# churchill-lab/alntools

Hardware: AMD Instinct MI355X
Metric: alignments/sec BAM->EC (100M PE reads, 8-hap) at 1/2/4/8 MI355X (higher is better)
Workload: dtype u32

## Files before the change

alntools_amd/csrc/ecb.hip:

```cpp
#include <hip/hip_runtime.h>

#include <algorithm>
#include <climits>
#include <cstddef>
#include <cstdarg>
#include <cstdio>
#include <cstring>
#include <cstdlib>
#include <memory>
#include <mutex>
#include <string>
#include <vector>

#include "../../include/ecb.h"

namespace {

typedef unsigned long long u64;
typedef unsigned int u32;
typedef unsigned short u16;

constexpr int TPB = 256;
constexpr u32 MAX_PROBE = 256;
constexpr u32 PENDING = 0xFFFFFFFFu;
// ... 8 lines not shown

constexpr u32 ERR_CONTRACT = 1u;
constexpr u32 ERR_RANGE = 2u;
constexpr u32 ERR_ARENA = 4u;
constexpr u32 ERR_QUEUE = 8u;
constexpr u32 ERR_INTERNAL = 16u;
constexpr u32 ERR_COUNT = 32u;

struct alignas(64) Slot {
    u64 lo;
    u32 n1;
    u32 off;
    u32 count;
    u32 first_inv;
    uint2 pair[INL];
};
static_assert(sizeof(Slot) == 64, "one EC per 64-byte line");
static_assert(offsetof(Slot, n1) == 8 && offsetof(Slot, off) == 12 && offsetof(Slot, count) == 16 && offsetof(Slot, first_inv) == 20,
              "k_count_bins reads {n1, off} and {count, first_inv} as 8-byte words");
struct Entry {
    u64 lo, reserved;
    u32 count, first_inv;
    u32 off, n;
};
static_assert(sizeof(Entry) == 32, "exchange format");

struct Counters {
    u64 all, valid;
    u64 arena_top;
    u64 n_queue;
    u64 n_queue_s[QSTRIPES];
    u64 n_ecs;
    u32 err;
    u32 full;
    u64 arena_reg[ARENA_REGIONS];
    u64 next_slice;
    u64 n_mismatch;
    u32 last_rid, pad_;
    u64 n_probe_tiles;
};

__host__ __device__ __forceinline__ u32 arena_regions(u64 arena_cap) { return (u32)(arena_cap >> 16 >= ARENA_REGIONS ? ARENA_REGIONS : (arena_cap >> 16 ? arena_cap >> 16 : 1)); }
__device__ __forceinline__ u64 arena_alloc(Counters* ctr, u64 arena_cap, u32 n, u32 hint) {
    const u32 R = arena_regions(arena_cap);
    const u64 per = arena_cap / R;
    for (u32 t = 0; t < R; ++t) {
        const u32 r = (hint + t) % R;
        const u64 at = atomicAdd(&ctr->arena_reg[r], (u64)n);
        if (at + n <= (u64)(r + 1) * per) return at;
    }
    return ~0ull;
}

__device__ __forceinline__ u32 fmix32(u32 h) {
    h ^= h >> 16; h *= 0x85EBCA6Bu;
    h ^= h >> 13; h *= 0xC2B2AE35u;
    h ^= h >> 16;
    return h;
}
__device__ __forceinline__ u64 pair_hash64(u32 locus, u32 mask) {
    const u32 h0 = fmix32(locus * 0x9E3779B1u + mask * 0x85EBCA77u + 0x7F4A7C15u);
    const u32 h1 = fmix32((h0 ^ locus) * 0xC2B2AE3Du + mask);
    return ((u64)h1 << 32) | h0;
}
__device__ __forceinline__ u64 finish_hash(u64 s0, u32 n) { return (s0 + ((u64)n << 32) + n) | 1ull; }

__device__ __forceinline__ bool rec_valid(u32 hf) {
    if (hf & 0x4u) return false;
    if (hf & 0x1u) {
        if ((hf & 0x80u) || !(hf & 0x2u) || (hf & (ECB_FLAG_MATE_OTHER_REF | ECB_FLAG_NEXT_POS_NEG))) return false;
    }
    return true;
}

enum { ST_NONE = 0, ST_LOOK, ST_HIT, ST_CREATED, ST_PENDING, ST_FULL, ST_OTHER, ST_STUCK };
enum { CMP_EQUAL = 0, CMP_DIFFERENT, CMP_INCOMPLETE, CMP_UNSURE };
struct SlotView { u32 n, off; uint2 p[INL]; };

__device__ __forceinline__ u64 fresh64(u64* p) { return atomicOr(p, 0ull); }
__device__ __forceinline__ void store_wt64(u64* p, u64 v) { __hip_atomic_store(p, v, __ATOMIC_RELAXED, __HIP_MEMORY_SCOPE_AGENT); }
__device__ __forceinline__ u64 pack2(uint2 v) { return ((u64)v.y << 32) | v.x; }
__device__ __forceinline__ uint2 unpack2(u64 v) { return make_uint2((u32)v, (u32)(v >> 32)); }
__device__ __forceinline__ void publish_key(Slot* s, u32 n1, u32 off) { store_wt64(reinterpret_cast<u64*>(&s->n1), ((u64)off << 32) | n1); }
__device__ __forceinline__ uint2 key_pair(const Slot& s, const uint2* arena, u32 i) { return i < INL ? s.pair[i] : arena[(u64)s.off + (i - INL)]; }
__device__ __forceinline__ uint2 key_pair_fresh(Slot* s, uint2* arena, u32 off, u32 i) {
    return unpack2(fresh64(reinterpret_cast<u64*>(i < INL ? &s->pair[i] : arena + ((u64)off + (i - INL)))));
}

__device__ __forceinline__ SlotView make_view(uint4 a, uint4 b, uint4 c, uint4 d) {
    SlotView v;
    v.n = a.z - 1u; v.off = a.w;
    v.p[0] = make_uint2(b.z, b.w); v.p[1] = make_uint2(c.x, c.y); v.p[2] = make_uint2(c.z, c.w);
    v.p[3] = make_uint2(d.x, d.y); v.p[4] = make_uint2(d.z, d.w);
    return v;
}
constexpr u32 RANKED_MAX = 16;
template <class F>
__device__ __forceinline__ void ranked_pairs(const SlotView& v, const uint2* arena, F&& emit) {
    const u32 sn = v.n;
    u32 X[RANKED_MAX], Y[RANKED_MAX];
#pragma unroll
    for (u32 i = 0; i < INL; ++i) { X[i] = i < sn ? v.p[i].x : 0xFFFFFFFFu; Y[i] = v.p[i].y; }
    if (sn <= INL) {
#pragma unroll
        for (u32 i = 0; i < INL; ++i) {
            u32 r = 0;
#pragma unroll
            for (u32 j = 0; j < INL; ++j) r += X[j] < X[i] ? 1u : 0u;
            if (i < sn) emit(r, X[i], Y[i]);
        }
    } else {
#pragma unroll
        for (u32 k = 0; k < RANKED_MAX - INL; ++k) {
            const uint2 t = INL + k < sn ? arena[(u64)v.off + k] : make_uint2(0xFFFFFFFFu, 0u);
            X[INL + k] = t.x; Y[INL + k] = t.y;
        }
#pragma unroll
        for (u32 i = 0; i < RANKED_MAX; ++i) {
            u32 r = 0;
#pragma unroll
            for (u32 j = 0; j < RANKED_MAX; ++j) r += X[j] < X[i] ? 1u : 0u;
            if (i < sn) emit(r, X[i], Y[i]);
        }
    }
}
constexpr u32 BIG_LDS = 2048;
template <class F>
__device__ __forceinline__ void ranked_pairs_wave(const Slot& s, const uint2* arena, u32 sn, u32* sx, u32 lane, F&& emit) {
    const bool in_lds = sn <= BIG_LDS;
    if (in_lds) {
        for (u32 i = lane; i < sn; i += 64) sx[i] = key_pair(s, arena, i).x;
        __builtin_amdgcn_fence(__ATOMIC_ACQ_REL, "wavefront");
        __builtin_amdgcn_wave_barrier();
    }
    for (u32 i = lane; i < sn; i += 64) {
        const uint2 pi = key_pair(s, arena, i);
        u32 r = 0;
        if (in_lds) {
            u32 j = 0;
            for (; j + 4u <= sn; j += 4u) {
                const uint4 v = *reinterpret_cast<const uint4*>(&sx[j]);
                r += (v.x < pi.x ? 1u : 0u) + (v.y < pi.x ? 1u : 0u) + (v.z < pi.x ? 1u : 0u) + (v.w < pi.x ? 1u : 0u);
            }
            for (; j < sn; ++j) r += sx[j] < pi.x ? 1u : 0u;
        } else {
            for (u32 j = 0; j < sn; ++j) r += key_pair(s, arena, j).x < pi.x;
        }
        emit(r, pi.x, pi.y);
    }
    if (in_lds) {
        __builtin_amdgcn_fence(__ATOMIC_ACQ_REL, "wavefront");
        __builtin_amdgcn_wave_barrier();
    }
}
template <class Cmp>
__device__ __forceinline__ int table_lookup(Slot* table, u64 cap_mask, u64 lo, u64& j, u32& probes, const Cmp& cmp, u32 abl = 0u, u32* first_inv_seen = nullptr) {
    for (; probes < MAX_PROBE; ++probes, j = (j + 1) & cap_mask) {
        Slot* s = table + j;
        const uint4* q = reinterpret_cast<const uint4*>(s);
        if (first_inv_seen) *first_inv_seen = 0u;
        uint4 a = q[0], b = a, c = a, d = a;
        if (!(abl & 16u)) { b = q[1]; c = q[2]; d = q[3]; }
        u64 clo = ((u64)a.y << 32) | a.x;
        if (clo == 0ull) {
            clo = atomicCAS(&s->lo, 0ull, lo);
            if (clo == 0ull) return ST_CREATED;
// ... 2283 lines not shown
int verify_pass(ecb_handle* h, const StreamPlan& P, const u32* d_rid, const u32* d_loc, const u32* d_hf, u64 n, u32 prev_rid, u64* n_long, u32 tw) {
    RCCHK(launch_stream(h, SV_VERIFY, P, d_rid, d_loc, d_hf, nullptr, n, prev_rid, nullptr, 0, 0));
    RCCHK(sync_counters(h));
    return run_deferred(h, d_rid, d_loc, d_hf, n, true, tw, n_long);
}
int verify_batch(ecb_handle* h, const u32* d_rid, const u32* d_loc, const u32* d_hf, u64 n, u32 prev_rid, u64* n_mismatch, u64* n_long, u32 tw = 512u) {
    StreamPlan P;
    RCCHK(plan_stream(h, n, &P, SV_VERIFY));
    u64 nq = 0;
    if (const int rc = verify_pass(h, P, d_rid, d_loc, d_hf, n, prev_rid, &nq, tw); rc != ECB_OK) {
        if (h->hctr.err) {
            const std::string refusal = h->err;
            HIPCHK(h, hipMemsetAsync(&h->ctr->err, 0, sizeof(u32), h->stream));
            HIPCHK(h, hipMemsetAsync(&h->ctr->n_queue, 0, (1 + QSTRIPES) * sizeof(u64), h->stream));
            h->hctr.err = 0; h->hctr.n_queue = 0;
            h->err = refusal;
        }
        return rc;
    }
    *n_mismatch = h->hctr.n_mismatch;
    *n_long = nq;
    HIPCHK(h, hipMemsetAsync(&h->ctr->n_queue, 0, (1 + QSTRIPES) * sizeof(u64), h->stream));
    h->hctr.n_queue = 0;
    return ECB_OK;
}

int build_batch(ecb_handle* h, const u32* d_rid, const u32* d_loc, const u32* d_hf, const int* d_pos, u64 n, u32 tw, bool* launched) {
    if (n == 0) return ECB_OK;
    const bool hinted = h->reads_hint != 0;
    u32 last_rid = 0;
    u64 reads_after = std::max<u64>(h->reads_hint, h->run.n_reads);
    if (!hinted) {
        HIPCHK(h, hipMemcpyAsync(&last_rid, d_rid + rec_at(n - 1, tw), sizeof(u32), hipMemcpyDeviceToHost, h->stream));
        HIPCHK(h, hipStreamSynchronize(h->stream));
        reads_after = (u64)(u32)(last_rid + 1u);
        if (reads_after < h->run.n_reads) return fail(h, ECB_ERR_CONTRACT, "read_id went backwards across pushes");
    }
    RCCHK(ensure_read_slot(h, reads_after));
    h->run.reads_hi = reads_after;
    while (h->n_ecs() * 2 > h->cap) { RCCHK(grow_table(h, h->cap * 4)); }
    const StreamVariant v = pick_variant(h, n);
    StreamPlan P;
    RCCHK(plan_stream(h, n, &P, v));
    u64* timing = nullptr;
#ifdef ECB_TIMING
    HIPCHK(h, hipMalloc(&timing, 8 * sizeof(u64)));
    HIPCHK(h, hipMemset(timing, 0, 8 * sizeof(u64)));
#endif
    h->ctr_synced = false;
    *launched = true;
    const u64 probe_before = h->hctr.n_probe_tiles;
    int rc = ECB_OK;
    for (u32 launch = 0;; ++launch) {
        rc = launch_stream(h, v, P, d_rid, d_loc, d_hf, d_pos, n, h->run.prev_rid, d_rid + rec_at(n - 1, tw), launch, launch ? 0 : n, timing);
        if (rc != ECB_OK) break;
        rc = sync_counters(h);
        if (h->prof) {
            float ms = 0; hipEventElapsedTime(&ms, h->ev0, h->ev1);
            h->prof_ms += ms; h->prof_launches += 1;
        }
        if (rc != ECB_OK) break;
        const bool parked = h->hctr.full != 0;
        rc = run_deferred(h, d_rid, d_loc, d_hf, n, false, tw);
        if (rc != ECB_OK) break;
        if (!parked) break;
        rc = grow_table(h, h->cap * 4);
        if (rc != ECB_OK) break;
    }
#ifdef ECB_TIMING
    {
        u64 t[8];
        hipMemcpy(t, timing, sizeof(t), hipMemcpyDeviceToHost); hipFree(timing);
        static const char* nm[8] = {"(a) filter+heads", "tile decisions", "prefetch issue+clear+geometry", "(b) LDS tables", "hash entries", "(c) lookup", "publish/settle/slot stores", "-"};
        u64 tot = 0; for (int i = 0; i < 7; ++i) tot += t[i];
        fprintf(stderr, "[ecb timing] %llu waves, clocks per wave:", (unsigned long long)P.slices);
        for (int i = 0; i < 7; ++i) fprintf(stderr, "  %s %.0f (%.1f%%)", nm[i], (double)t[i] / P.slices, 100.0 * t[i] / std::max<u64>(tot, 1));
        fprintf(stderr, "  tile visits on the probe-on path %llu of %llu tiles", (unsigned long long)t[7], (unsigned long long)((n + WT - 1) / WT));
        fprintf(stderr, "\n");
    }
#endif
    RCCHK(rc);
    {
        const u64 tiles = (n + WT - 1) / WT, on_path = h->hctr.n_probe_tiles - probe_before;
        if (on_path * 4 > tiles) h->par_stream = true; else if (on_path * 16 < tiles) h->par_stream = false;
    }
    if (h->prof) h->prof_records += n;
    if (h->cfg.flags & ECB_F_VERIFY) {
        u64 bad = 0, nl = 0;
        RCCHK(verify_batch(h, d_rid, d_loc, d_hf, n, h->run.prev_rid, &bad, &nl, tw));
        h->run.n_mismatch += bad;
        if (bad) return fail(h, ECB_ERR_VERIFY, "exactness pass: %llu read(s) of this batch sit in an EC whose key is not their target set", (unsigned long long)bad);
    }
    if (hinted) {
        last_rid = h->hctr.last_rid;
        reads_after = (u64)(u32)(last_rid + 1u);
        if (reads_after < h->run.n_reads) return fail(h, ECB_ERR_CONTRACT, "read_id went backwards across pushes");
    }
    h->run.prev_rid = last_rid;
    h->run.n_reads = reads_after;
    h->run.records_pushed += n;
    return ECB_OK;
}
int process_batch(ecb_handle* h, const u32* d_rid, const u32* d_loc, const u32* d_hf, const int* d_pos, u64 n, u32 tw = 512u) {
    bool launched = false;
    const int rc = build_batch(h, d_rid, d_loc, d_hf, d_pos, n, tw, &launched);
    return launched ? run_refused(h, rc) : rc;
}

int ensure_staging(ecb_handle* h, u64 need) {
    if (need <= h->st_cap) return ECB_OK;
    h->st_loc = h->st_hf = nullptr; h->st_pos = nullptr; h->st_cap = 0;
    const u64 cap = std::max<u64>(need, h->cfg.max_batch_records);
    const u64 stride = (cap * sizeof(u32) + (2ull << 20) - 1) / (2ull << 20) * (2ull << 20) / sizeof(u32);
    const bool rg = (h->cfg.flags & ECB_F_RANGES) != 0;
    HIPCHK(h, h->st_rid.alloc((rg ? 4 : 3) * stride * sizeof(u32)));
    h->st_cap = cap;
    h->st_loc = h->st_rid + stride; h->st_hf = h->st_rid + 2 * stride;
    if (rg) h->st_pos = reinterpret_cast<int*>(h->st_rid + 3 * stride);
    return ECB_OK;
}

int stage_and_process(ecb_handle* h, const u32* rid, const u32* loc, const u32* hf, const int* pos, u64 m) {
    const u64 nc = h->run.c_rid.size();
    const u64 n = nc + m;
    if (!n) return ECB_OK;
    RCCHK(ensure_staging(h, n));
    const bool rg = (h->cfg.flags & ECB_F_RANGES) != 0;
    const struct { void* st; const void *carry, *window; } streams[4] = {
        {h->st_rid, h->run.c_rid.data(), rid}, {h->st_loc, h->run.c_loc.data(), loc}, {h->st_hf, h->run.c_hf.data(), hf}, {h->st_pos, h->run.c_pos.data(), pos}};
    for (int w = 0; w < 2; ++w)
        for (int i = 0; i < (rg ? 4 : 3) && (w ? m : nc); ++i)
            HIPCHK(h, hipMemcpyAsync((u32*)streams[i].st + (w ? nc : 0), w ? streams[i].window : streams[i].carry, (w ? m : nc) * 4, hipMemcpyHostToDevice, h->stream));
    HIPCHK(h, hipStreamSynchronize(h->stream));
    h->run.c_rid.clear(); h->run.c_loc.clear(); h->run.c_hf.clear(); h->run.c_pos.clear();
    return process_batch(h, h->st_rid, h->st_loc, h->st_hf, rg ? h->st_pos : nullptr, n);
}

int excl_scan_dev(ecb_handle* h, const u32* in, u64 n, u32* out, u64* d_total, u32 stride = 1, u32* last32 = nullptr) {
    u32* sums = nullptr;
    POOL(h, P_SUMS, sums, scan_words(n));
    HIPCHK(h, scan_launch(h->stream, in, n, out, sums, d_total, stride, last32));
    return ECB_OK;
}
int excl_scan(ecb_handle* h, const u32* in, u64 n, u32* out, u64* total) {
    u64* d_tot = nullptr;
    POOL(h, P_TOTALS, d_tot, 8);
    RCCHK(excl_scan_dev(h, in, n, out, d_tot + 7));
    HIPCHK(h, hipMemcpyAsync(total, d_tot + 7, sizeof(u64), hipMemcpyDeviceToHost, h->stream));
    HIPCHK(h, hipStreamSynchronize(h->stream));
    return ECB_OK;
}

struct SortBufs {
    u64* k[2];
    u32* v[2];
    int at = 0;
    u64* keys() const { return k[at]; }
    u32* vals() const { return v[at]; }
    u64* spare_keys() const { return k[at ^ 1]; }
    u32* spare_vals() const { return v[at ^ 1]; }
};
struct SortScratch { u32 *hist, *offs; u64* d_word; };
inline u64 rs_tiles(u64 n) { return std::max<u64>(1, (n + RS_TILE - 1) / RS_TILE); }
constexpr u64 RS_AUX_WORDS = 2 * RS_MAX_PASSES * 256 + 64;
inline u64 rs_words(u64 n) { return std::max<u64>(256 * rs_tiles(n), RS_AUX_WORDS); }
hipError_t radix_sort_pairs64(hipStream_t st, SortBufs& b, u64 n, const SortScratch& sc, u64 bit_mask = ~0ull) {
    b.at = 0;
// ... 3120 lines not shown
```

alntools_amd/csrc/k_stream.inc:

```
constexpr bool KS_SHORT = ECB_KS_SHORT != 0;
#ifndef ECB_KS_PAR
#define ECB_KS_PAR 0
#endif
constexpr bool KS_PAR = ECB_KS_PAR != 0;
static_assert(!(KS_PAR && KS_SHORT), "one or the other");
constexpr u32 KBITS = KS_SHORT ? 25 : 26;
constexpr u32 KMASK = (1u << KBITS) - 1u;
constexpr int WMAXR = KS_SHORT ? 128 : 64;
#ifndef ECB_WAVES_PER_SIMD
#define ECB_WAVES_PER_SIMD 5
#endif
#ifndef ECB_LGMAX
#define ECB_LGMAX 6
#endif
#ifndef ECB_EST_MUL
#define ECB_EST_MUL 4
#endif
constexpr int WAVES_PER_SIMD = KS_SHORT ? 4 : ECB_WAVES_PER_SIMD;
constexpr int LGMAX = KS_SHORT ? 7 : ECB_LGMAX;
static_assert(LGMAX >= 0 && (1 << LGMAX) <= WMAXR && KBITS + LGMAX <= 32, "a read's index within the pass: the bits of an LDS key above KBITS");
constexpr int CMAX = KS_SHORT ? 64 : 80;
#ifndef ECB_TSLOTS
#define ECB_TSLOTS (ECB_WAVES_PER_SIMD > 4 ? 640 : 896)
#endif
constexpr int TSLOTS = KS_SHORT ? 1280 : ECB_TSLOTS;
constexpr int TBASE = KS_SHORT ? 1024 : 512;
constexpr int TAB_BYTES = KS_SHORT ? TSLOTS * 4 + 2048 : TSLOTS * 8;
static_assert((TSLOTS == 896 || TSLOTS == 640 || TSLOTS == 1280) && WT + CMAX < TSLOTS && TAB_BYTES % (16 * 64) == 0 && (!KS_SHORT || TSLOTS <= 2048), "home regions / a free slot / clear loop");
constexpr u32 SBITS = KS_SHORT ? 11 : 10;
constexpr u32 SMASK = (1u << SBITS) - 1u;
static_assert(TSLOTS <= (1 << SBITS) && (KS_SHORT || SBITS + LGMAX <= 16), "ent[] packs slot | read << SBITS into 16 bits (128 reads: the slot alone, the read is in the table's key)");
struct alignas(16) WaveLds {
#ifdef ECB_TAB_INTERLEAVED
    uint2 tab[TSLOTS];
#else
    u32 tkey[TSLOTS];
    u32 tmask[KS_SHORT ? 512 : TSLOTS];
#endif
    u64 acc[WMAXR];
    uint2 carry[CMAX];
    unsigned short ent[WT + CMAX];
    unsigned short npair[WMAXR];
    u32 ws[8];
};
static_assert(sizeof(WaveLds) * NWAVE * WAVES_PER_SIMD <= 160 * 1024, "WAVES_PER_SIMD workgroups per CU");
__device__ __forceinline__ u64 ws_get64(const WaveLds& L, int i) {
    const u32 lo = (u32)__builtin_amdgcn_readfirstlane((int)L.ws[i]), hi = (u32)__builtin_amdgcn_readfirstlane((int)L.ws[i + 1]);
    return ((u64)hi << 32) | lo;
}
__device__ __forceinline__ void ws_put64(WaveLds& L, int i, u64 v, u32 lane) { if (lane == 0) { L.ws[i] = (u32)v; L.ws[i + 1] = (u32)(v >> 32); } }
#ifdef ECB_TAB_INTERLEAVED
__device__ __forceinline__ u32* tab_key(WaveLds& L, u32 q) { return &L.tab[q].x; }
__device__ __forceinline__ void tab_or(WaveLds& L, u32 q, u32 bits) { static_assert(!KS_SHORT, "byte masks: split arrays only"); atomicOr(&L.tab[q].y, bits); }
__device__ __forceinline__ uint2 tab_get(const WaveLds& L, u32 q) { return L.tab[q]; }
__device__ __forceinline__ uint4* tab_base(WaveLds& L) { return reinterpret_cast<uint4*>(L.tab); }
#else
__device__ __forceinline__ u32* tab_key(WaveLds& L, u32 q) { return &L.tkey[q]; }
__device__ __forceinline__ void tab_or(WaveLds& L, u32 q, u32 bits) {
    if constexpr (KS_SHORT) atomicOr(&L.tmask[q >> 2], bits << ((q & 3u) * 8u)); else atomicOr(&L.tmask[q], bits);
}
__device__ __forceinline__ uint2 tab_get(const WaveLds& L, u32 q) {
    if constexpr (KS_SHORT) return make_uint2(L.tkey[q], (L.tmask[q >> 2] >> ((q & 3u) * 8u)) & 0xFFu);
    else return make_uint2(L.tkey[q], L.tmask[q]);
}
__device__ __forceinline__ uint4* tab_base(WaveLds& L) { return reinterpret_cast<uint4*>(L.tkey); }
#endif
struct HomeGeo { u32 fmul, g; };
__device__ __forceinline__ u32 pack_lgf(u32 lg) {
    const u32 g = (u32)(KS_SHORT ? 10 : 9) - lg;
    u32 x = 1u << 16, f = 0;
#pragma unroll
    for (int i = 0; i < 6; ++i) { f += x; x >>= g; }
    return f | (lg << 24);
}
__device__ __forceinline__ HomeGeo home_geo(u32 lgf) {
    HomeGeo H;
    H.fmul = lgf;
    H.g = (u32)(KS_SHORT ? 10 : 9) - (lgf >> 24);
    return H;
}
__device__ __forceinline__ u32 home_off(u32 key, const HomeGeo& H) { return __builtin_amdgcn_ubfe(__umul24(key, H.fmul), 16u, H.g); }
__device__ __forceinline__ u32 next_slot(u32 key, u32 q, u32 it) {
    if (it == 0u) return __umulhi(key * 0x9E3779B1u, (u32)TSLOTS);
    constexpr u32 ODD_FACTOR = TSLOTS == 896 ? 7u : 5u;
    u32 s = 1u + 2u * ((key >> 5) & 31u);
    if (s % ODD_FACTOR == 0u) s += 2u;
    q += s;
    return q >= (u32)TSLOTS ? q - (u32)TSLOTS : q;
}
__device__ __forceinline__ u32 probe_slot(u32 key, u32 it) {
    u32 q = __umulhi(key * 0x9E3779B1u, (u32)TSLOTS);
    if (it != 0u) {
        constexpr u32 ODD_FACTOR = TSLOTS == 896 ? 7u : 5u;
        u32 s = 1u + 2u * ((key >> 5) & 31u);
        if (s % ODD_FACTOR == 0u) s += 2u;
        q = (q + it * s) % (u32)TSLOTS;
    }
    return q;
}

struct LdsSetCmp {
    const WaveLds* L;
    u32 home, tag, np;
// ... 106 lines not shown
            const u32 key = tag | (pr.x + 1u);
            u32 q = home + home_off(pr.x + 1u, H);
            bool found = false;
            for (u32 it = 0; it < (u32)TSLOTS; ++it) {
                const uint2 t = tab_get(*L, q);
                if (t.x == key) { found = t.y == pr.y; break; }
                if (t.x == 0u) break;
                q = next_slot(key, q, it);
            }
            if (!found) return CMP_DIFFERENT;
        }
        return CMP_EQUAL;
    }
};

template <bool VERIFY, bool RANGES = false>
__global__ __launch_bounds__(TPB, RANGES ? (WAVES_PER_SIMD < 4 ? WAVES_PER_SIMD : 4) : WAVES_PER_SIMD) void k_stream(StreamArgs A) {
    __shared__ WaveLds wl[NWAVE];
    const u32 lane = threadIdx.x & 63u, w = threadIdx.x >> 6;
    WaveLds& L = wl[w];
    const u64 pw = (u64)blockIdx.x * NWAVE + w;
    const StreamCold* const C = A.cold;
    static_assert(WT == 512, "tile index = record index >> 9");
    u32 my_valid = 0, my_new = 0;
    u32 bad = 0;
    if (lane == 0) L.ws[7] = 0u;
    if (!VERIFY && lane == 0) { const u64* wa = C->wave_arena; const u64 ca = wa[2 * pw]; L.ws[2] = (u32)ca; L.ws[3] = (u32)(ca >> 32); L.ws[4] = (u32)wa[2 * pw + 1]; }
#ifdef ECB_TIMING
    u64 tacc[8] = {0, 0, 0, 0, 0, 0, 0, 0}, tlast = __builtin_readcyclecounter();
#endif
    auto clear_pass = [&](u32 ln) {
        uint4* z = tab_base(L);
        u32 zz;
        asm volatile("v_mov_b32 %0, 0" : "=v"(zz));
        const uint4 zv = make_uint4(zz, zz, zz, zz);
#pragma unroll
        for (int t = 0; t < TAB_BYTES / (16 * 64); ++t) z[t * 64 + ln] = zv;
        if constexpr (KS_SHORT) { reinterpret_cast<uint4*>(L.acc)[ln] = zv; reinterpret_cast<u32*>(L.npair)[ln] = zz; }
        else { *reinterpret_cast<uint2*>(&L.acc[ln]) = make_uint2(zz, zz); L.npair[ln] = (unsigned short)zz; }
    };
    clear_pass(lane);
    wave_sync();
  for (;;) {
    u32 wid = 0;
    if (lane == 0) wid = (u32)atomicAdd(&A.ctr->next_slice, 1ull);
    wid = (u32)__builtin_amdgcn_readfirstlane((int)wid);
    const u64 chunk = C->chunk;
    const u64 c0 = (u64)wid * chunk;
    if (c0 >= A.n) break;
    const u64 c1 = min(c0 + chunk, A.n);
    const u64 p = C->resume[2 * (u64)wid], counted0 = C->resume[2 * (u64)wid + 1];
    if (p >= A.n || p == ~0ull) continue;
    u32 tix = (u32)(p >> 9);
    const u32 c1t = (u32)((c1 + (u64)(WT - 1)) >> 9);
    const u32 last_t = (u32)((A.n - 1) >> 9);
    const u32 last_rel = (u32)(A.n - ((u64)last_t << 9));
    const u32 counted_t = (u32)((counted0 + (u64)(WT - 1)) >> 9);
    int p_rel = (int)(p - ((u64)tix << 9));
    u32 prev = p == 0 ? C->prev_rid : A.rid[rec_at(p - 1, A_TW(A))];
    u32 pb = prev + 1u, npend = 0, n_ent = 0;
    ws_put64(L, 5, p, lane);
    bool open = false;
    u32 carry_n = 0;
    u32 lgf = pack_lgf(LGMAX);
    bool revisit = false;
    TileRegs R;
    load_tile(A, (u64)tix << 9, min(((u64)tix << 9) + (u64)WT, A.n), lane, R);
    int r_pos[RANGES ? RPL : 1];
    if constexpr (RANGES) load_pos(A.pos, (u64)tix << 9, min(((u64)tix << 9) + (u64)WT, A.n), lane, r_pos);
    u32 parked = __hip_atomic_load(&A.ctr->full, __ATOMIC_RELAXED, __HIP_MEMORY_SCOPE_AGENT);
    asm volatile("" : "+v"(parked));
    bool slice_done = false;

    while (!slice_done) {
        if (__builtin_amdgcn_readfirstlane((int)parked)) break;
        u32 ln = lane;
        asm volatile("" : "+v"(ln));
        tix = (u32)__builtin_amdgcn_readfirstlane((int)tix);
        prev = (u32)__builtin_amdgcn_readfirstlane((int)prev);
        pb = (u32)__builtin_amdgcn_readfirstlane((int)pb);
        npend = (u32)__builtin_amdgcn_readfirstlane((int)npend);
        n_ent = (u32)__builtin_amdgcn_readfirstlane((int)n_ent);
        lgf = (u32)__builtin_amdgcn_readfirstlane((int)lgf);
        const u32 lg = lgf >> 24;
        const u32 gp = ((u32)TBASE >> lg) + (TSLOTS == 896 ? (256u >> lg) : 0u) + ((u32)(TBASE / 4) >> lg);
        const HomeGeo HG = home_geo(lgf);
        bool do_flush = false, again = false, more = false;
        bool preflush = false;
        bool taken = false;
        u32 parked_next = parked;
        u32 last_pos = 0xFFFFFFFFu;
        u32 last_rid = prev;
        u32 est = 64;
        const bool ends = tix == last_t;
        const bool own = tix < c1t;
        const int te_rel = ends ? (int)last_rel : WT;
        const bool count_tile = own && tix >= counted_t && !revisit;
        const bool plain = p_rel == 0 && te_rel == WT;
        u32 r_key[RPL], r_bit[RPL];
        u32 m_act = 0, m_head = 0;
        const u32 lim = own ? (1u << lg) : (open ? npend + 1u : 0u);
        const u32 rid_first = (u32)__builtin_amdgcn_readfirstlane((int)R.rr[0]), rid_last = (u32)__builtin_amdgcn_readlane((int)R.rr[RPL - 1], 63);
        const bool all_mine = rid_first - pb < lim && rid_last - pb < lim && rid_last >= rid_first;
        {
#pragma unroll
            for (int g = 0; g < NG; ++g) {
                const int i0 = g * 256 + 4 * (int)ln;
                const u32 up = lane_above(R.rr[4 * g + 3]);
                const u32 wrap = g == 0 ? prev : (u32)__builtin_amdgcn_readlane((int)R.rr[4 * (g > 0 ? g - 1 : 0) + 3], 63);
                u32 in4 = 0xFu, te4 = 0xFu;
                if (!plain) {
                    te4 = (1u << clamp04(te_rel - i0, 0, 4)) - 1u;
                    in4 = te4 & ~((1u << clamp04(p_rel - i0, 0, 4)) - 1u);
                }
                const u32 prev0 = ln == 0 ? wrap : up;
                u32 ok4 = 0, head4 = 0, hap_or = 0, mine4 = 0;
#pragma unroll
                for (int j = 3; j >= 0; --j) {
                    const u32 f = R.hh[4 * g + j];
                    const u32 pair_ok = ((f & 0x3082u) ^ 0x2u) - 1u;
                    const u32 ok31 = ~(f << 29) & (~(f << 31) | pair_ok);
                    ok4 = __builtin_amdgcn_alignbit(ok4, ok31, 31);
                }
#pragma unroll
                for (int par = 0; par < 2; ++par) {
                    if (__ballot((ok4 & (par ? 0xAu : 0x5u)) != 0u) != 0ull) {
#pragma unroll
                        for (int j = par; j < 4; j += 2) {
                            const int k = 4 * g + j;
                            const u32 f = R.hh[k];
                            const u32 step = R.rr[k] - (j == 0 ? prev0 : R.rr[k > 0 ? k - 1 : 0]);
                            const u32 relx = R.rr[k] - pb;
                            const u32 t = R.ll[k] + 1u;
                            r_key[k] = t | (relx << KBITS);
                            r_bit[k] = 1u << ((f >> ECB_HAP_SHIFT) & 31u);
                            hap_or |= ((t & ~KMASK) | f) & (u32)((int)(ok4 << (31 - j)) >> 31);
                            head4 |= (step & 1u) << j;
                            if (!all_mine) mine4 |= (relx < lim ? 1u : 0u) << j;
                        }
                        if constexpr (RANGES) {
                            if (!revisit) {
                                const u32 nl = C->n_loci, nh = C->n_haps;
                                int2* const rng = A.rng;
                                u32 sl[2]; int2 cur[2]; bool go[2];
#pragma unroll
                                for (int j = par; j < 4; j += 2) {
                                    const int k = 4 * g + j;
                                    const u32 lc = R.ll[k], hap = (R.hh[k] >> ECB_HAP_SHIFT) & 0xFFu;
                                    go[j >> 1] = ((ok4 >> j) & 1u) && lc < nl && hap < nh;
                                    sl[j >> 1] = lc * nh + hap;
                                    cur[j >> 1] = make_int2(0, 0);
                                    if (go[j >> 1]) cur[j >> 1] = rng[sl[j >> 1]];
                                }
#pragma unroll
                                for (int j = par; j < 4; j += 2) {
                                    const int ps = r_pos[RANGES ? 4 * g + j : 0];
                                    if (go[j >> 1] && ps < cur[j >> 1].x) atomicMin(&rng[sl[j >> 1]].x, ps);
                                    if (go[j >> 1] && ps > cur[j >> 1].y) atomicMax(&rng[sl[j >> 1]].y, ps);
                                }
                            }
                        }
                    } else {
#pragma unroll
                        for (int j = par; j < 4; j += 2) {
                            asm volatile("" : "=v"(r_key[4 * g + j])); asm volatile("" : "=v"(r_bit[4 * g + j]));
                        }
                    }
                }
                const u32 big = (u32)(R.rr[4 * g + 3] - prev0 != (u32)__popc(head4));
                if (count_tile) my_valid += __popc(ok4 & te4);
                ok4 &= in4; head4 &= in4;
                bad |= ((p_rel == 0 ? big : 0u) | (head4 & ~ok4)) ? ERR_CONTRACT : 0u;
                bad |= (hap_or >> (ECB_HAP_SHIFT + (KS_SHORT ? 3 : 5))) ? ERR_RANGE : 0u;
                m_act |= (all_mine ? ok4 : (ok4 & mine4)) << (4 * g); m_head |= head4 << (4 * g);
            }
        }
        TICK(0);
        if (__ballot(bad != 0u)) break;
        const u32 cnts = wave_sum((u32)__popc(m_head) | ((u32)__popc(m_act) << 16));
        const u32 nheads = cnts & 0xFFFFu, n_mine = cnts >> 16;
        last_rid = (u32)__builtin_amdgcn_readlane((int)R.rr[RPL - 1], 63);
        const u32 o1 = open ? 1u : 0u;
        const u32 n_new = own ? (prev + 1u + nheads) - (pb + npend + o1) : 0u;
        const u32 n_in = o1 + n_new;
        est = n_in;
        if (n_ent + carry_n + n_mine > (u32)(WT + CMAX)) { preflush = true; do_flush = true; }
        else {
        if (own) {
            if (npend + n_in > (1u << lg)) { again = true; npend = 1u << lg; open = false; }
            else if (n_in) { npend += ends ? n_in : n_in - 1u; open = !ends; }
        } else if (open && (nheads || ends)) { npend += 1u; open = false; }
        more = !ends && (tix + 1u < c1t || open);
        TICK(1);
        if (more || again) {
            u32 lp = ln;
#pragma unroll
            for (int k = 0; k < RPL; ++k) asm volatile("" : "+v"(lp) : "v"(r_key[k]), "v"(r_bit[k]));
            asm volatile("" : "+v"(lp) : "v"(m_act), "v"(m_head), "v"(bad), "v"(my_valid));
            const u64 nt = (u64)(again ? tix : tix + 1u) << 9;
            load_tile(A, nt, min(nt + (u64)WT, A.n), lp, R);
            if constexpr (RANGES) load_pos(A.pos, nt, min(nt + (u64)WT, A.n), lp, r_pos);
            parked_next = __hip_atomic_load(&A.ctr->full, __ATOMIC_RELAXED, __HIP_MEMORY_SCOPE_AGENT);
        }
        if (!again) {
            const u64 h1 = __ballot((m_head >> 4) != 0u), h0 = __ballot((m_head & 15u) != 0u);
            if (h1 | h0) {
                const u32 l = 63u - (u32)__builtin_clzll(h1 ? h1 : h0);
                const u32 bits = (u32)__builtin_amdgcn_readlane((int)m_head, (int)l);
                const u32 k = 31u - (u32)__builtin_clz(h1 ? bits & 0xF0u : bits & 0xFu);
                last_pos = (k & 3u) + (k >> 2) * 256u + 4u * l;
            }
            if (open && last_pos != 0xFFFFFFFFu) ws_put64(L, 0, ((u64)tix << 9) + last_pos, ln);
        }

        TICK(2);
        if (!ABL(A, 1u)) {
            const bool cin = carry_n != 0u;
            u32 q[RPL + 1], old[RPL + 1], act = m_act;
            u32 cb = 0;
            u32 c_key = 0, c_bit = 0;
            if (cin && ln < carry_n) { const uint2 cv = L.carry[ln]; c_key = cv.x; c_bit = cv.y; act |= 1u << RPL; }
#pragma unroll
            for (int h = 0; h < 2; ++h) {
                const u32 hmask = h ? 0x0AAu : 0x155u;
                if (__ballot((act & hmask) != 0u) == 0ull) continue;
#pragma unroll
                for (int k = h; k <= RPL; k += 2) {
                    const u32 key = k < RPL ? r_key[k < RPL ? k : 0] : c_key;
                    q[k] = (act >> k & 1u) ? (key >> KBITS) * gp + home_off(key, HG) : ln;
                }
#pragma unroll
                for (int k = h; k <= RPL; k += 2)
                    old[k] = atomicCAS(tab_key(L, q[k]), (act >> k & 1u) ? 0u : 0xFFFFFFFFu, k < RPL ? r_key[k < RPL ? k : 0] : c_key);
#pragma unroll
                for (int k = h; k <= RPL; k += 2) {
                    const u32 key = k < RPL ? r_key[k < RPL ? k : 0] : c_key, bit = k < RPL ? r_bit[k < RPL ? k : 0] : c_bit;
                    const bool on = act >> k & 1u;
                    const bool made = on && old[k] == 0u;
                    const bool hit = made || (on && old[k] == key);
                    cb |= (on && !hit ? 1u : 0u) << k;
                    tab_or(L, q[k], hit ? bit : 0u);
                    const u64 mm = __ballot(made);
                    if (made) L.ent[n_ent + __builtin_amdgcn_mbcnt_hi((u32)(mm >> 32), __builtin_amdgcn_mbcnt_lo((u32)mm, 0u))] =
                        (unsigned short)(KS_SHORT ? q[k] : (q[k] | ((key >> KBITS) << SBITS)));
                    n_ent += (u32)__popcll(mm);
                }
            }
            const bool anyc = cb != 0u;
            if (__ballot(anyc) || (cin && carry_n > 64u)) {
#ifdef ECB_TIMING
                tacc[7] += 1;
#endif
                if (ln == 0) L.ws[7] += 1u;
                u32 lo_ = 0, hi_ = 0;
                bool from_home = cin && carry_n > 64u;
                if (from_home) { lo_ = 64u; hi_ = carry_n; }
                for (;;) {
                    if (!from_home) {
                        if (!__ballot(cb != 0u)) break;
                        wave_sync();
                        u32 n_st = 0;
#pragma unroll
                        for (int k = 0; k <= RPL; ++k) {
                            const bool c = cb >> k & 1u;
                            const u64 mm = __ballot(c);
                            if (!mm) continue;
                            const u32 at = n_st + __builtin_amdgcn_mbcnt_hi((u32)(mm >> 32), __builtin_amdgcn_mbcnt_lo((u32)mm, 0u));
                            if (c && at < (u32)CMAX) {
                                const u32 key = k < RPL ? r_key[k < RPL ? k : 0] : c_key, bit = k < RPL ? r_bit[k < RPL ? k : 0] : c_bit;
                                L.carry[at] = make_uint2(key, bit);
                                cb &= ~(1u << k);
                            }
                            n_st = min(n_st + (u32)__popcll(mm), (u32)CMAX);
                        }
                        lo_ = 0u; hi_ = n_st;
                        wave_sync();
                    }
                    for (u32 base = lo_; base < hi_; base += 64u) {
                        const bool have = base + ln < hi_;
                        const uint2 rec = L.carry[have ? base + ln : 0u];
                        bool todo = have, made = false;
                        u32 it = from_home ? 0xFFFFFFFFu : 0u, qq = 0;
                        while (__ballot(todo)) {
                            if (todo) {
// ... 20 lines not shown

        bool giant = false;
        u32 new_carry = 0;
        if (do_flush) {
            wave_sync();
            u32 cn = 0;
            const u32 rl_last = npend;
            const bool keep = open;
            for (u32 e0 = 0; e0 < n_ent; e0 += 64) {
                const u32 e = e0 + ln;
                const bool have = e < n_ent;
                const u32 en = have ? L.ent[e] : 0u, qq = en & SMASK;
                const uint2 en2 = tab_get(L, qq);
                const u32 rl = KS_SHORT ? en2.x >> KBITS : en >> SBITS;
                const bool kept = have && keep && rl == rl_last;
                if (have && !kept) {
                    atomicAdd(&L.acc[rl], pair_hash64((en2.x & KMASK) - 1u, en2.y));
                    atomicAdd(reinterpret_cast<u32*>(&L.npair[rl & ~1u]), (rl & 1u) ? 0x10000u : 1u);
                }
                if (keep) {
                    const u64 mm = __ballot(kept);
                    const u32 at = cn + __builtin_amdgcn_mbcnt_hi((u32)(mm >> 32), __builtin_amdgcn_mbcnt_lo((u32)mm, 0u));
                    if (kept && at < (u32)CMAX) L.carry[at] = make_uint2(en2.x & KMASK, en2.y);
                    cn += (u32)__popcll(mm);
                }
            }
            if (keep) { new_carry = cn; giant = cn > (u32)CMAX; }
            wave_sync();

            TICK(4);
            const u32 nhalf = KS_SHORT ? ((u32)__builtin_amdgcn_readfirstlane((int)npend) + 63u) >> 6 : 1u;
          for (u32 half = 0; half < nhalf; ++half) {
            u64 j = 0;
            u32 st = ST_NONE, probes = 0, np = 0, fseen = 0;
            u64 lo = 0;
            const u32 rx = KS_SHORT ? ln + (half << 6) : ln;
            const bool on = rx < npend && !ABL(A, 3u);
            const u32 rd = pb + rx;
            LdsSetCmp cmp;
            cmp.L = &L; cmp.cold = C; cmp.home = rx * gp; cmp.H = HG; cmp.tag = rx << KBITS; cmp.np = 0;
            if (on) {
                np = L.npair[rx];
                cmp.np = np;
                lo = finish_hash(L.acc[rx], np);
                j = lo & A.cap_mask;
                if ((u64)rd >= A.reads_hi) bad |= ERR_CONTRACT;
                else st = ST_LOOK;
            }
            if (VERIFY) {
                if (st == ST_LOOK) {
                    const u32 sl = A.read_slot[rd];
                    bool same = false;
                    if (sl != PENDING) {
                        const uint4* q = reinterpret_cast<const uint4*>(A.table + sl);
                        const uint4 a = q[0], b = q[1], c = q[2], d = q[3];
                        if (a.z != 0u && a.z != DEAD_KEY) {
                            int r = cmp.quick(make_view(a, b, c, d));
                            if (r == CMP_UNSURE) r = cmp.full(A.table + sl, a.z - 1u, a.w);
                            same = r == CMP_EQUAL;
                        }
                    }
                    if (!same) my_new += 1;
                }
                parked = parked_next; taken = true;
                        } else {
                for (u32 round = 0;; ++round) {
                    if (st == ST_LOOK) {
                        if (ABL(A, 64u)) { st = ST_HIT; fseen = 0xFFFFFFFFu; }
                        else if (ABL(A, 4u)) st = ST_HIT;
                        else st = table_lookup(A.table, A.cap_mask, lo, j, probes, cmp, ABL(A, 24u), &fseen);
                    }
                    if (round == 0u && half == 0u) {
                        TICK(5);
                        parked = parked_next; taken = true;
                    #pragma unroll
                        for (int k = 0; k < RPL; ++k) {
                            asm volatile("" : "+v"(R.rr[k])); asm volatile("" : "+v"(R.ll[k])); asm volatile("" : "+v"(R.hh[k]));
                            if constexpr (RANGES) asm volatile("" : "+v"(r_pos[k]));
                        }
                        asm volatile("" : "+v"(parked));
                    }
                    const u64 cmask = __ballot(st == ST_CREATED);
                    if (cmask) {
                        const bool cr = st == ST_CREATED;
                        const u32 want = cr && np > INL ? np - INL : 0u;
                        u32 off = 0;
                        if (__ballot(want != 0u)) {
                            const u32 incl = wave_incl_scan(want);
                            const u32 total = (u32)__builtin_amdgcn_readlane((int)incl, 63);
                            u64 chunk_at = ws_get64(L, 2);
                            u32 chunk_left = (u32)__builtin_amdgcn_readfirstlane((int)L.ws[4]);
                            if (total > chunk_left) {
                                const u32 take = max(total, ARENA_CHUNK);
                                u64 at = 0;
                                if (ln == 0) at = arena_alloc(A.ctr, C->arena_cap, take, (u32)pw);
                                chunk_at = ((u64)(u32)__builtin_amdgcn_readfirstlane((int)(u32)(at >> 32)) << 32) | (u32)__builtin_amdgcn_readfirstlane((int)(u32)at);
                                chunk_left = take;
                                if (chunk_at == ~0ull) { bad |= ERR_ARENA; chunk_left = 0; }
                            }
                            if (!(bad & ERR_ARENA)) {
                                off = (u32)(chunk_at + (incl - want));
                                chunk_at += total; chunk_left -= total;
                            }
                            ws_put64(L, 2, chunk_at, ln);
                            if (ln == 0) L.ws[4] = chunk_left;
                        }
                        const bool dead = (bad & ERR_ARENA) != 0u;
                        const u32 j32 = (u32)j;
                        uint2* const arena = C->arena;
                        if (!dead) for (u32 e0 = 0; e0 < n_ent; e0 += 64) {
                            const u32 e = e0 + ln;
                            const u32 en = e < n_ent ? L.ent[e] : 0u, qq = en & SMASK;
                            const u32 rl = KS_SHORT ? tab_get(L, qq).x >> KBITS : en >> SBITS;
                            const u32 o = __shfl(off, rl & 63u), jj = __shfl(j32, rl & 63u);
                            if (e < n_ent && (!KS_SHORT || (rl >> 6) == half) && (cmask >> (rl & 63u) & 1ull) && !ABL(A, 32u)) {
                                const u32 was = atomicSub(reinterpret_cast<u32*>(&L.npair[rl & ~1u]), (rl & 1u) ? 0x10000u : 1u);
                                const u32 pos = ((rl & 1u) ? was >> 16 : was & 0xFFFFu) - 1u;
                                uint2* dst = pos < INL ? &A.table[jj].pair[pos] : arena + ((u64)o + (pos - INL));
                                const uint2 en2 = tab_get(L, qq);
                                store_wt64(reinterpret_cast<u64*>(dst), pack2(make_uint2((en2.x & KMASK) - 1u, en2.y)));
                            }
                        }
                        if (cr) { publish_key(A.table + j, dead ? DEAD_KEY : np + 1u, off); st = ST_HIT; }
                        my_new += (u32)__popcll(cmask);
                    }
                    if (!__ballot(st == ST_PENDING)) break;
                    if (round >= 64u) { if (st == ST_PENDING) { bad |= ERR_INTERNAL; st = ST_NONE; } break; }
                    if (st == ST_PENDING) {
                        const int r = table_settle(A.table + j, cmp);
                        if (r == ST_HIT) st = ST_HIT;
                        else if (r == ST_STUCK) { bad |= ERR_INTERNAL; st = ST_NONE; atomicExch(&A.ctr->full, 1u); }
                        else { j = (j + 1) & A.cap_mask; ++probes; st = ST_LOOK; }
                    }
                }
                if (st == ST_FULL) {
                    atomicExch(&A.ctr->full, 1u);
                    queue_defer(A.ctr, C, tile_head(A.rid, (u64)wid * C->chunk, min(((u64)tix << 9) + (u64)WT, A.n), rd, A_TW(A)));
                } else if (st == ST_HIT) {
                    A.read_slot[rd] = (u32)j;
                    if (~rd > fseen) atomicMax(&A.table[j].first_inv, ~rd);
                }
            }
          }
            wave_sync();
            clear_pass(ln);
            pb += npend; npend = 0; n_ent = 0;
            const u32 e4 = min(est * (u32)ECB_EST_MUL, 1u << LGMAX);
            lgf = pack_lgf(e4 > 1u ? 32u - (u32)__builtin_clz(e4 - 1u) : 0u);
            if (open) {
                if (!giant) carry_n = new_carry;
                else {
                    if (ln == 0) {
                        queue_defer(A.ctr, C, ws_get64(L, 0));
                    }
                    open = false; pb += 1u;
                }
            }
            ws_put64(L, 5, open ? ws_get64(L, 0) : (u64)((preflush || again) ? tix : tix + 1u) << 9, ln);
            wave_sync();
            TICK(6);
        }
        if (preflush) { revisit = true; continue; }
        if (!taken) {
            parked = parked_next;
        #pragma unroll
            for (int k = 0; k < RPL; ++k) {
                asm volatile("" : "+v"(R.rr[k])); asm volatile("" : "+v"(R.ll[k])); asm volatile("" : "+v"(R.hh[k]));
                if constexpr (RANGES) asm volatile("" : "+v"(r_pos[k]));
            }
            asm volatile("" : "+v"(parked));
        }
        if (again) { revisit = true; continue; }
        revisit = false; p_rel = 0;
        prev = last_rid;
        slice_done = !more;
        tix += 1u;
    }
    u64 p_out = ws_get64(L, 5);
    const u64 counted = max(counted0, min((u64)(revisit ? tix + 1u : tix) << 9, c1));
    const bool stopped = __ballot(bad != 0u) || __builtin_amdgcn_readfirstlane((int)parked);
    if (__ballot(bad != 0u)) { if (bad) atomicOr(&A.ctr->err, bad); p_out = ~0ull; }
    else if (slice_done) p_out = ~0ull;
    if (lane == 0) { u64* rs = C->resume; rs[2 * (u64)wid] = p_out; rs[2 * (u64)wid + 1] = counted; }
    if (stopped) break;
  }
    const u32 wa = (u32)__builtin_amdgcn_readfirstlane((int)L.ws[7]), wv = wave_sum(my_valid);
    const u32 wn = VERIFY ? wave_sum(my_new) : my_new;
#ifdef ECB_TIMING
    if (lane == 0 && C->timing) for (int i = 0; i < 8; ++i) atomicAdd(C->timing + i, tacc[i]);
#endif
    if (lane == 0) { u32* wc = C->wave_counts; wc[3 * pw] = wa; wc[3 * pw + 1] = wv; wc[3 * pw + 2] = wn; }
    if (!VERIFY && lane == 0) { u64* wav = C->wave_arena; wav[2 * pw] = ((u64)L.ws[3] << 32) | L.ws[2]; wav[2 * pw + 1] = L.ws[4]; }
}
```

Before: 374.3 billion.

## Write founder EC slots as whole-line buffer stores and shorten tail tile loads

When a newly created EC has at most INL pairs and all its pairs sit in the wave's LDS home region, the wave gathers the key and pairs with bpermute and writes the entire slot line with four 128-bit buffer stores. This replaces the per-entry atomic LDS counter and the scattered 64-bit global stores, and it also publishes the key in the same step. Separately, tiles past the owned range are first loaded as a short 64-record tail. A full tile is revisited only if more is needed, which cuts over-read past the slice boundary. The changes add complexity in the publish ordering, since the whole line is written non-atomically, and add extra ballot loops per founder.

```diff
diff --git a/alntools_amd/csrc/ecb.hip b/alntools_amd/csrc/ecb.hip
--- a/alntools_amd/csrc/ecb.hip
+++ b/alntools_amd/csrc/ecb.hip
@@ -114,6 +114,12 @@
 __device__ __forceinline__ u64 pack2(uint2 v) { return ((u64)v.y << 32) | v.x; }
 __device__ __forceinline__ uint2 unpack2(u64 v) { return make_uint2((u32)v, (u32)(v >> 32)); }
 __device__ __forceinline__ void publish_key(Slot* s, u32 n1, u32 off) { store_wt64(reinterpret_cast<u64*>(&s->n1), ((u64)off << 32) | n1); }
+__device__ __forceinline__ void found_line(Slot* s, u32 x, u32 y, u32 z, u32 w, u32 lane) {
+    typedef unsigned int u32x4 __attribute__((ext_vector_type(4)));
+    const __amdgpu_buffer_rsrc_t rs = __builtin_amdgcn_make_buffer_rsrc(s, 0, (int)sizeof(Slot), 0x00020000);
+    u32x4 v; v.x = x; v.y = y; v.z = z; v.w = w;
+    if (lane < 4u) __builtin_amdgcn_raw_buffer_store_b128(v, rs, lane * 16u, 0, 16);
+}
 __device__ __forceinline__ uint2 key_pair(const Slot& s, const uint2* arena, u32 i) { return i < INL ? s.pair[i] : arena[(u64)s.off + (i - INL)]; }
 __device__ __forceinline__ uint2 key_pair_fresh(Slot* s, uint2* arena, u32 off, u32 i) {
     return unpack2(fresh64(reinterpret_cast<u64*>(i < INL ? &s->pair[i] : arena + ((u64)off + (i - INL)))));
@@ -2563,7 +2569,11 @@
     RCCHK(rc);
     {
         const u64 tiles = (n + WT - 1) / WT, on_path = h->hctr.n_probe_tiles - probe_before;
+#ifdef ECB_COUNT_FOUNDERS
+        fprintf(stderr, "ecb founders: %llu served by a line store (plus tiles on the probe-on path), %llu ECs in the table\n", (unsigned long long)on_path, (unsigned long long)h->hctr.n_ecs);
+#else
         if (on_path * 4 > tiles) h->par_stream = true; else if (on_path * 16 < tiles) h->par_stream = false;
+#endif
     }
     if (h->prof) h->prof_records += n;
     if (h->cfg.flags & ECB_F_VERIFY) {
diff --git a/alntools_amd/csrc/k_stream.inc b/alntools_amd/csrc/k_stream.inc
--- a/alntools_amd/csrc/k_stream.inc
+++ b/alntools_amd/csrc/k_stream.inc
@@ -19,6 +19,12 @@
 constexpr int WAVES_PER_SIMD = KS_SHORT ? 4 : ECB_WAVES_PER_SIMD;
 constexpr int LGMAX = KS_SHORT ? 7 : ECB_LGMAX;
 static_assert(LGMAX >= 0 && (1 << LGMAX) <= WMAXR && KBITS + LGMAX <= 32, "a read's index within the pass: the bits of an LDS key above KBITS");
+#ifndef ECB_FOUND_LINE
+#define ECB_FOUND_LINE 1
+#endif
+constexpr bool FOUND_LINE = ECB_FOUND_LINE != 0 && !KS_SHORT && !KS_PAR;
+constexpr bool TAIL_SHORT = !KS_SHORT;
+constexpr int TAILW = 64;
 constexpr int CMAX = KS_SHORT ? 64 : 80;
 #ifndef ECB_TSLOTS
 #define ECB_TSLOTS (ECB_WAVES_PER_SIMD > 4 ? 640 : 896)
@@ -291,6 +297,7 @@
         npend = (u32)__builtin_amdgcn_readfirstlane((int)npend);
         n_ent = (u32)__builtin_amdgcn_readfirstlane((int)n_ent);
         lgf = (u32)__builtin_amdgcn_readfirstlane((int)lgf);
+        if constexpr (TAIL_SHORT) p_rel = __builtin_amdgcn_readfirstlane(p_rel);
         const u32 lg = lgf >> 24;
         const u32 gp = ((u32)TBASE >> lg) + (TSLOTS == 896 ? (256u >> lg) : 0u) + ((u32)(TBASE / 4) >> lg);
         const HomeGeo HG = home_geo(lgf);
@@ -301,8 +308,9 @@
         u32 last_pos = 0xFFFFFFFFu;
         u32 last_rid = prev;
         u32 est = 64;
+        const bool own = tix < c1t;
+        const bool tail = TAIL_SHORT && !own && p_rel == 0;
         const bool ends = tix == last_t;
-        const bool own = tix < c1t;
         const int te_rel = ends ? (int)last_rel : WT;
         const bool count_tile = own && tix >= counted_t && !revisit;
         const bool plain = p_rel == 0 && te_rel == WT;
@@ -406,9 +414,10 @@
 #pragma unroll
             for (int k = 0; k < RPL; ++k) asm volatile("" : "+v"(lp) : "v"(r_key[k]), "v"(r_bit[k]));
             asm volatile("" : "+v"(lp) : "v"(m_act), "v"(m_head), "v"(bad), "v"(my_valid));
-            const u64 nt = (u64)(again ? tix : tix + 1u) << 9;
-            load_tile(A, nt, min(nt + (u64)WT, A.n), lp, R);
-            if constexpr (RANGES) load_pos(A.pos, nt, min(nt + (u64)WT, A.n), lp, r_pos);
+            const u64 nt = (u64)((again || tail) ? tix : tix + 1u) << 9;
+            const u64 nte = min(nt + (u64)((!TAIL_SHORT || again || tail || tix + 1u < c1t || tix + 1u == last_t) ? WT : TAILW), A.n);
+            load_tile(A, nt, nte, lp, R);
+            if constexpr (RANGES) load_pos(A.pos, nt, nte, lp, r_pos);
             parked_next = __hip_atomic_load(&A.ctr->full, __ATOMIC_RELAXED, __HIP_MEMORY_SCOPE_AGENT);
         }
         if (!again) {
@@ -595,6 +604,45 @@
                     }
                     const u64 cmask = __ballot(st == ST_CREATED);
                     if (cmask) {
+                        u64 fmask = 0ull;
+                        if constexpr (FOUND_LINE && !RANGES) {
+                            const bool cand = st == ST_CREATED && np <= INL && !ABL(A, 32u);
+                            if (gp <= 64u) for (u64 fm = __ballot(cand); fm; fm &= fm - 1ull) {
+                                const u32 f = (u32)__builtin_ctzll(fm);
+                                const u32 frx = KS_SHORT ? f + (half << 6) : f;
+                                const u32 fnp = (u32)__builtin_amdgcn_readlane((int)np, (int)f);
+                                const uint2 t = tab_get(L, frx * gp + (ln < gp ? ln : 0u));
+                                const bool mine = ln < gp && t.x != 0u && (t.x >> KBITS) == frx;
+                                u64 m = __ballot(mine);
+                                if ((u32)__popcll(m) != fnp) continue;
+                                fmask |= 1ull << f;
+                                u32 src[INL];
+#pragma unroll
+                                for (u32 r = 0; r < INL; ++r) { src[r] = m ? (u32)__builtin_ctzll(m) : 0u; m &= m - 1ull; }
+                                const u32 kx = (t.x & KMASK) - 1u, ky = t.y;
+                                const u32 sa = ln == 2u ? src[1] : src[3], sb = ln == 1u ? src[0] : ln == 2u ? src[2] : src[4];
+                                const bool va = ln >= 2u && 2u * ln - 3u < fnp, vb = ln >= 1u && 2u * ln - 2u < fnp;
+                                const u32 ax = (u32)__builtin_amdgcn_ds_bpermute((int)(sa << 2), (int)kx), ay = (u32)__builtin_amdgcn_ds_bpermute((int)(sa << 2), (int)ky);
+                                const u32 bx = (u32)__builtin_amdgcn_ds_bpermute((int)(sb << 2), (int)kx), by = (u32)__builtin_amdgcn_ds_bpermute((int)(sb << 2), (int)ky);
+                                const u32 flo = (u32)__builtin_amdgcn_readlane((int)(u32)lo, (int)f), fhi = (u32)__builtin_amdgcn_readlane((int)(u32)(lo >> 32), (int)f);
+                                const u64 fj = ((u64)(u32)__builtin_amdgcn_readlane((int)(u32)(j >> 32), (int)f) << 32) | (u32)__builtin_amdgcn_readlane((int)(u32)j, (int)f);
+                                const u32 w0 = ln == 0u ? flo : va ? ax : 0u;
+                                const u32 w1 = ln == 0u ? fhi : ln == 1u ? ~(pb + frx) : va ? ay : 0u;
+                                const u32 w2 = ln == 0u ? fnp + 1u : vb ? bx : 0u;
+                                const u32 w3 = vb ? by : 0u;
+                                found_line(A.table + fj, w0, w1, w2, w3, ln);
+                            }
+#ifdef ECB_COUNT_FOUNDERS
+                            if (ln == 0) L.ws[7] += (u32)__popcll(fmask);
+#endif
+                            if (fmask >> ln & 1ull) {
+                                st = ST_HIT;
+#ifndef ECB_FOUND_ATOMIC
+                                fseen = ~rd;
+#endif
+                            }
+                        }
+                        const u64 smask = cmask & ~fmask;
                         const bool cr = st == ST_CREATED;
                         const u32 want = cr && np > INL ? np - INL : 0u;
                         u32 off = 0;
@@ -621,12 +669,12 @@
                         const bool dead = (bad & ERR_ARENA) != 0u;
                         const u32 j32 = (u32)j;
                         uint2* const arena = C->arena;
-                        if (!dead) for (u32 e0 = 0; e0 < n_ent; e0 += 64) {
+                        if (!dead && smask) for (u32 e0 = 0; e0 < n_ent; e0 += 64) {
                             const u32 e = e0 + ln;
                             const u32 en = e < n_ent ? L.ent[e] : 0u, qq = en & SMASK;
                             const u32 rl = KS_SHORT ? tab_get(L, qq).x >> KBITS : en >> SBITS;
                             const u32 o = __shfl(off, rl & 63u), jj = __shfl(j32, rl & 63u);
-                            if (e < n_ent && (!KS_SHORT || (rl >> 6) == half) && (cmask >> (rl & 63u) & 1ull) && !ABL(A, 32u)) {
+                            if (e < n_ent && (!KS_SHORT || (rl >> 6) == half) && (smask >> (rl & 63u) & 1ull) && !ABL(A, 32u)) {
                                 const u32 was = atomicSub(reinterpret_cast<u32*>(&L.npair[rl & ~1u]), (rl & 1u) ? 0x10000u : 1u);
                                 const u32 pos = ((rl & 1u) ? was >> 16 : was & 0xFFFFu) - 1u;
                                 uint2* dst = pos < INL ? &A.table[jj].pair[pos] : arena + ((u64)o + (pos - INL));
@@ -684,6 +732,7 @@
             asm volatile("" : "+v"(parked));
         }
         if (again) { revisit = true; continue; }
+        if (TAIL_SHORT && more && p_rel == 0 && tix >= c1t) { revisit = false; p_rel = TAILW; continue; }
         revisit = false; p_rel = 0;
         prev = last_rid;
         slice_done = !more;
```

Result: slower. 367.4 billion (-1.8%).
